# samuel-watson/glmmrMCML

Hardware: AMD Instinct MI355X
Metric: MCML iters/sec x m chains (simlik evals/sec) (higher is better)
Workload: dtype f64

## Files before the change

glmmrmcml_amd/csrc/debug_hooks.hip:

```cpp
#include "dgemm_mfma.h"
#include "dgemm_dl.h"
#include "dgemm_band.h"

using namespace mcml;

extern "C" int glmmr_mcml_dbg_dgemm(int M, int N, int K, const double* A, int lda,
                                    const double* B, int ldb, int b_nmajor,
                                    double alpha, double beta, double* C, int ldc,
                                    int lower_only, int force_tile)
{
    int ndev = 0;
    if (hipGetDeviceCount(&ndev) != hipSuccess || ndev == 0) {
        set_error("no HIP device: libglmmr_mcml_hip has no CPU fallback");
        return MCML_ENODEVICE;
    }
    hipStream_t s = nullptr;
    DevMat dA, dB, dC;
    if (force_tile == 40) {
        MCML_REQUIRE(!b_nmajor && !lower_only, "dbg_dgemm: the direct-to-LDS kernel takes a K-major B and all tiles");
        const int kpad = round_up(K, 32);
        MCML_TRY(dA.alloc(M, K, 32));
        MCML_HIP(hipMemset(dA.d(), 0, sizeof(double) * (size_t)dA.ld * dA.cols_alloc));
        MCML_HIP(hipMemcpy2D(dA.d(), sizeof(double) * dA.ld, A, sizeof(double) * lda, sizeof(double) * M, K, hipMemcpyHostToDevice));
        MCML_TRY(dB.alloc(kpad, N));
        MCML_HIP(hipMemset(dB.d(), 0, sizeof(double) * (size_t)dB.ld * N));
        MCML_HIP(hipMemcpy2D(dB.d(), sizeof(double) * dB.ld, B, sizeof(double) * ldb, sizeof(double) * K, N, hipMemcpyHostToDevice));
        MCML_TRY(upload_matrix(dC, C, M, N, ldc, s));
        MCML_REQUIRE(dlds_applicable(M, N, K, dA.d(), dA.ld, dA.cols_alloc, dB.d(), dB.ld), "dbg_dgemm: operands do not meet the direct-to-LDS contract");
        EpiAxpby epi2{dC.d(), dC.ld, alpha, beta};
        MCML_TRY(launch_gemm_dlds(s, M, N, K, dA.d(), dA.ld, dB.d(), dB.ld, epi2));
        MCML_TRY(download_matrix(C, ldc, dC.d(), dC.ld, M, N, s));
        return MCML_OK;
    }
    MCML_TRY(upload_matrix(dA, A, M, K, lda, s));
    if (b_nmajor) MCML_TRY(upload_matrix(dB, B, N, K, ldb, s));
    else MCML_TRY(upload_matrix(dB, B, K, N, ldb, s));
    MCML_TRY(upload_matrix(dC, C, M, N, ldc, s));
    EpiAxpby epi{dC.d(), dC.ld, alpha, beta};
    int rc;
    if (force_tile >= 20)
        rc = b_nmajor ? launch_gemm_dl<true>(s, M, N, K, dA.d(), dA.ld, dB.d(), dB.ld, epi, lower_only != 0, force_tile - 19)
                      : launch_gemm_dl<false>(s, M, N, K, dA.d(), dA.ld, dB.d(), dB.ld, epi, lower_only != 0, force_tile - 19);
    else
        rc = b_nmajor ? launch_gemm<true>(s, M, N, K, dA.d(), dA.ld, dB.d(), dB.ld, epi, lower_only != 0, force_tile)
                      : launch_gemm<false>(s, M, N, K, dA.d(), dA.ld, dB.d(), dB.ld, epi, lower_only != 0, force_tile);
    MCML_TRY(rc);
    MCML_TRY(download_matrix(C, ldc, dC.d(), dC.ld, M, N, s));
    return MCML_OK;
}

extern "C" int glmmr_mcml_dbg_dgemm_bench2(int M, int N, int K, int b_nmajor, int iters, int force_tile,
                                           int lower_only, double beta, double* ms_per_launch);
extern "C" int glmmr_mcml_dbg_dgemm_bench(int M, int N, int K, int b_nmajor, int iters,
                                          int force_tile, double* ms_per_launch)
{
    return glmmr_mcml_dbg_dgemm_bench2(M, N, K, b_nmajor, iters, force_tile, 0, 0.0, ms_per_launch);
}

extern "C" int glmmr_mcml_dbg_dgemm_bench2(int M, int N, int K, int b_nmajor, int iters, int force_tile,
                                           int lower_only, double beta, double* ms_per_launch)
{
    int ndev = 0;
    if (hipGetDeviceCount(&ndev) != hipSuccess || ndev == 0) {
        set_error("no HIP device: libglmmr_mcml_hip has no CPU fallback");
        return MCML_ENODEVICE;
    }
    hipStream_t s = nullptr;
    std::vector<double> hA((size_t)M * K), hB((size_t)K * N), hC((size_t)M * N, 0.0);
    uint64_t x = 88172645463325252ULL;
    auto rnd = [&]() { x ^= x << 13; x ^= x >> 7; x ^= x << 17; return (double)(x >> 11) / 9007199254740992.0 * 2 - 1; };
    for (auto& v : hA) v = rnd();
    for (auto& v : hB) v = rnd();
    DevMat dA, dB, dC;
    MCML_TRY(upload_matrix(dA, hA.data(), M, K, M, s));
    if (b_nmajor) MCML_TRY(upload_matrix(dB, hB.data(), N, K, N, s));
    else MCML_TRY(upload_matrix(dB, hB.data(), K, N, K, s));
    MCML_TRY(upload_matrix(dC, hC.data(), M, N, M, s));
    EpiAxpby epi{dC.d(), dC.ld, beta != 0.0 ? 1e-3 : 1.0, beta};
    const bool lo = lower_only != 0;
    auto go = [&]() {
        if (force_tile >= 20)
            return b_nmajor ? launch_gemm_dl<true>(s, M, N, K, dA.d(), dA.ld, dB.d(), dB.ld, epi, lo, force_tile - 19)
                            : launch_gemm_dl<false>(s, M, N, K, dA.d(), dA.ld, dB.d(), dB.ld, epi, lo, force_tile - 19);
        return b_nmajor ? launch_gemm<true>(s, M, N, K, dA.d(), dA.ld, dB.d(), dB.ld, epi, lo, force_tile)
                        : launch_gemm<false>(s, M, N, K, dA.d(), dA.ld, dB.d(), dB.ld, epi, lo, force_tile);
    };
    for (int i = 0; i < 3; i++) MCML_TRY(go());
    hipEvent_t e0, e1;
    MCML_HIP(hipEventCreate(&e0));
    MCML_HIP(hipEventCreate(&e1));
    MCML_HIP(hipEventRecord(e0, s));
    for (int i = 0; i < iters; i++) MCML_TRY(go());
    MCML_HIP(hipEventRecord(e1, s));
    MCML_HIP(hipEventSynchronize(e1));
    float ms = 0;
    MCML_HIP(hipEventElapsedTime(&ms, e0, e1));
    *ms_per_launch = ms / iters;
    (void)hipEventDestroy(e0);
    (void)hipEventDestroy(e1);
    return MCML_OK;
}

extern "C" int glmmr_mcml_dbg_dgemm_band(int M, int N, int K, const double* A, int lda, const double* B, int ldb,
                                         double* C, int ldc, int* tiles_executed)
{
    int ndev = 0;
    if (hipGetDeviceCount(&ndev) != hipSuccess || ndev == 0) {
        set_error("no HIP device: libglmmr_mcml_hip has no CPU fallback");
        return MCML_ENODEVICE;
    }
    MCML_REQUIRE(M > 0 && N > 0 && K > 0 && A && B && C, "dbg_dgemm_band: bad argument");
    hipStream_t s = nullptr;
    DevMat dA, dB, dC;
    MCML_TRY(dA.alloc(M, K, 32));
    MCML_HIP(hipMemset(dA.d(), 0, sizeof(double) * (size_t)dA.ld * dA.cols_alloc));
    MCML_HIP(hipMemcpy2D(dA.d(), sizeof(double) * dA.ld, A, sizeof(double) * lda, sizeof(double) * M, K, hipMemcpyHostToDevice));
    MCML_TRY(dB.alloc(round_up(K, 32), N));
    MCML_HIP(hipMemset(dB.d(), 0, sizeof(double) * (size_t)dB.ld * N));
    MCML_HIP(hipMemcpy2D(dB.d(), sizeof(double) * dB.ld, B, sizeof(double) * ldb, sizeof(double) * K, N, hipMemcpyHostToDevice));
    MCML_TRY(dC.alloc(M, N));
    MCML_HIP(hipMemset(dC.d(), 0, sizeof(double) * (size_t)dC.ld * N));
    MCML_REQUIRE(dlds_applicable(M, N, K, dA.d(), dA.ld, dA.cols_alloc, dB.d(), dB.ld), "dbg_dgemm_band: contract");
    const int nbands = (M + BD_BM - 1) / BD_BM;
    DevBuf kr;
    MCML_TRY(kr.ensure(sizeof(int) * 2 * nbands));
    hipLaunchKernelGGL(k_band_ranges, dim3(nbands), dim3(256), 0, s, dA.d(), dA.ld, M, K, kr.as<int>());
    MCML_HIP(hipGetLastError());
    std::vector<int> hk(2 * nbands);
    MCML_HIP(hipMemcpy(hk.data(), kr.p, sizeof(int) * 2 * nbands, hipMemcpyDeviceToHost));
    BandPlan plan;
    plan.reset(M, K, hk);
    if (tiles_executed) *tiles_executed = (int)plan.tiles;
    EpiAxpby epi{dC.d(), dC.ld, 1.0, 0.0};
    MCML_TRY(launch_gemm_band(s, plan, N, dA.d(), dA.ld, dB.d(), dB.ld, epi));
    MCML_TRY(download_matrix(C, ldc, dC.d(), dC.ld, M, N, s));
    return MCML_OK;
}

extern "C" int glmmr_mcml_dbg_band_clocks(int M, int N, int iters, int mode, double* out3)
{
    int ndev = 0;
    if (hipGetDeviceCount(&ndev) != hipSuccess || ndev == 0) {
        set_error("no HIP device: libglmmr_mcml_hip has no CPU fallback");
        return MCML_ENODEVICE;
    }
    hipStream_t s = nullptr;
    if (getenv("GLMMR_MCML_DBG_STREAM")) MCML_HIP(hipStreamCreateWithFlags(&s, hipStreamNonBlocking));
    std::vector<double> hA((size_t)M * M, 0.0), hB((size_t)M * N);
    uint64_t x = 88172645463325252ULL;
    auto rnd = [&]() { x ^= x << 13; x ^= x >> 7; x ^= x << 17; return (double)(x >> 11) / 9007199254740992.0 * 2 - 1; };
    const bool cst = getenv("GLMMR_MCML_DBG_DATA") && !strcmp(getenv("GLMMR_MCML_DBG_DATA"), "const");
    const bool dec = getenv("GLMMR_MCML_DBG_DATA") && !strcmp(getenv("GLMMR_MCML_DBG_DATA"), "decay");
    for (int j = 0; j < M; ++j) for (int i = j; i < M; ++i) hA[i + (size_t)j * M] = cst ? 1.0 : dec ? rnd() * std::exp(-(double)(i - j) / 40.0) : rnd();
    for (auto& v : hB) v = cst ? 1.0 : rnd();
    DevMat dA, dB, dC;
    MCML_TRY(dA.alloc(M, M, 32));
    MCML_HIP(hipMemset(dA.d(), 0, sizeof(double) * (size_t)dA.ld * dA.cols_alloc));
    MCML_HIP(hipMemcpy2D(dA.d(), sizeof(double) * dA.ld, hA.data(), sizeof(double) * M, sizeof(double) * M, M, hipMemcpyHostToDevice));
    MCML_TRY(dB.alloc(round_up(M, 32), N));
    MCML_HIP(hipMemset(dB.d(), 0, sizeof(double) * (size_t)dB.ld * N));
    MCML_HIP(hipMemcpy2D(dB.d(), sizeof(double) * dB.ld, hB.data(), sizeof(double) * M, sizeof(double) * M, N, hipMemcpyHostToDevice));
    MCML_TRY(dC.alloc(M, N));
    const int nbands = (M + BD_BM - 1) / BD_BM;
    DevBuf kr, clk;
    MCML_TRY(kr.ensure(sizeof(int) * 2 * nbands));
    MCML_TRY(clk.ensure(16));
    MCML_HIP(hipMemset(clk.p, 0, 16));
    hipLaunchKernelGGL(k_band_ranges, dim3(nbands), dim3(256), 0, s, dA.d(), dA.ld, M, M, kr.as<int>());
    std::vector<int> hk(2 * nbands);
    MCML_HIP(hipMemcpy(hk.data(), kr.p, sizeof(int) * 2 * nbands, hipMemcpyDeviceToHost));
    BandPlan plan;
    plan.reset(M, M, hk);
    const double tiles = (double)plan.tiles;
    EpiAxpby epi{dC.d(), dC.ld, 1.0, 0.0};
    if (mode < 0) {
        for (int i = 0; i < 3; i++)
            MCML_TRY((launch_gemm_band<EpiAxpby, false>(s, plan, N, dA.d(), dA.ld, dB.d(), dB.ld, epi)));
        hipEvent_t f0, f1;
        MCML_HIP(hipEventCreate(&f0));
        MCML_HIP(hipEventCreate(&f1));
        MCML_HIP(hipEventRecord(f0, s));
        for (int i = 0; i < iters; i++)
// ... 190 lines not shown
```

glmmrmcml_amd/csrc/dgemm_dl.h:

```cpp
#pragma once
#include "dgemm_dlds.h"

namespace mcml {

template <int WTM, int WTN, int WM, int WN, bool BNMAJOR, int STAGES>
struct DlgCfg {
    static constexpr int BK = 16;
    static constexpr int NW = WM * WN, THREADS = 64 * NW;
    static constexpr int BM = 16 * WTM * WM, BN = 16 * WTN * WN;
    static constexpr int A_BYTES = BK * BM * 8, B_BYTES = BK * BN * 8;
    static constexpr int A_CHUNKS = A_BYTES / 1024, B_CHUNKS = B_BYTES / 1024;
    static constexpr int CHUNKS = A_CHUNKS + B_CHUNKS;
    static constexpr int PER = (CHUNKS + NW - 1) / NW;
    static constexpr int STAGE_BYTES = A_BYTES + B_BYTES;
    static constexpr size_t LDS_BYTES = (size_t)STAGES * STAGE_BYTES;
    static constexpr bool SWZ_A = (BM % 32) == 0;
    static constexpr bool SWZ_B = BNMAJOR && (BN % 32) == 0;
    static_assert(BM % 8 == 0 && BN % 8 == 0, "tile sides are multiples of 8 doubles");
    static_assert(LDS_BYTES <= 160 * 1024, "LDS ring does not fit");
    static_assert(PER * (STAGES - 1) <= 24, "vmcnt immediates in dl_wait_vm");
};

template <int N>
__device__ __forceinline__ void dl_wait_vm()
{
#define MCML_VM(n) else if constexpr (N == n) asm volatile("s_waitcnt vmcnt(" #n ")" ::: "memory");
    if constexpr (N <= 0) asm volatile("s_waitcnt vmcnt(0)" ::: "memory");
    MCML_VM(1) MCML_VM(2) MCML_VM(3) MCML_VM(4) MCML_VM(5) MCML_VM(6) MCML_VM(7) MCML_VM(8)
    MCML_VM(9) MCML_VM(10) MCML_VM(11) MCML_VM(12) MCML_VM(13) MCML_VM(14) MCML_VM(15) MCML_VM(16)
    MCML_VM(17) MCML_VM(18) MCML_VM(19) MCML_VM(20) MCML_VM(21) MCML_VM(22) MCML_VM(23) MCML_VM(24)
    else asm volatile("s_waitcnt vmcnt(0)" ::: "memory");
#undef MCML_VM
}

template <int PER, int MAXT>
__device__ __forceinline__ void dl_wait_leave(int tiles)
{
    if constexpr (MAXT <= 0) dl_wait_vm<0>();
    else {
        if (tiles >= MAXT) dl_wait_vm<PER * MAXT>();
        else dl_wait_leave<PER, MAXT - 1>(tiles);
    }
}

template <int WTM, int WTN, int WM, int WN, bool BNMAJOR, int STAGES, class Epi>
__global__ __launch_bounds__(64 * WM * WN) void dgemm_dl_kernel(GemmP p, Epi epi)
{
    using Cfg = DlgCfg<WTM, WTN, WM, WN, BNMAJOR, STAGES>;
    constexpr int BM = Cfg::BM, BN = Cfg::BN, BK = Cfg::BK, NW = Cfg::NW, PER = Cfg::PER;
    extern __shared__ __attribute__((aligned(16))) double smem[];
    char* lds = reinterpret_cast<char*>(smem);
    const int tid = threadIdx.x, lane = tid & 63, wave = __builtin_amdgcn_readfirstlane(tid >> 6);
    const int wr = wave / WN, wc = wave - wr * WN;

    const int nblk = gridDim.x;
    const int bid = blockIdx.x;
    const int q8 = nblk >> 3, r8 = nblk & 7, xcd = bid & 7;
    const int nid = (xcd < r8 ? xcd * (q8 + 1) : r8 * (q8 + 1) + (xcd - r8) * q8) + (bid >> 3);
    int bi, bj;
    if (p.lower_only) {
        int rem = nid;
        for (bi = 0; bi < p.gm; ++bi) {
            int nc = (bi * BM + BM - 1 + p.diag_shift) / BN + 1;
            if (nc > p.gn) nc = p.gn;
            if (rem < nc) break;
            rem -= nc;
        }
        bj = rem;
    } else {
        bi = nid / p.gn; bj = nid - bi * p.gn;
    }
    const int m0 = bi * BM, n0 = bj * BN;

    unsigned voff[PER]; int loff[PER]; bool isA[PER];
#pragma unroll
    for (int s = 0; s < PER; ++s) {
        int c = wave + NW * s;
        if (c >= Cfg::CHUNKS) c = wave;
        isA[s] = c < Cfg::A_CHUNKS;
        if (c < Cfg::A_CHUNKS) {
            const int o = c * 1024 + lane * 16;
            const int k = o / (BM * 8), pos = (o - k * BM * 8) >> 3;
            const int m = Cfg::SWZ_A ? ((((pos >> 4) ^ (k & 1)) << 4) | (pos & 15)) : pos;
            int gm = m0 + m;
            if (gm >= p.M) gm = 0;
            voff[s] = (unsigned)((gm + (size_t)k * p.lda) * 8);
            loff[s] = c * 1024;
        } else {
            const int cb = c - Cfg::A_CHUNKS;
            const int o = cb * 1024 + lane * 16;
            if (BNMAJOR) {
                const int k = o / (BN * 8), pos = (o - k * BN * 8) >> 3;
                const int n = Cfg::SWZ_B ? ((((pos >> 4) ^ (k & 1)) << 4) | (pos & 15)) : pos;
                int gn = n0 + n;
                if (gn >= p.N) gn = 0;
                voff[s] = (unsigned)((gn + (size_t)k * p.ldb) * 8);
            } else {
                const int q = o >> 4;
                const int kp = q / BN, n = q - kp * BN;
                int gn = n0 + n;
                if (gn >= p.N) gn = 0;
                voff[s] = (unsigned)((2 * kp + (size_t)gn * p.ldb) * 8);
            }
            loff[s] = Cfg::A_BYTES + cb * 1024;
        }
    }
    const size_t stepA = (size_t)BK * p.lda * 8, stepB = BNMAJOR ? (size_t)BK * p.ldb * 8 : (size_t)BK * 8;
    const int by = blockIdx.y;
    const char* sA = reinterpret_cast<const char*>(p.A + (size_t)by * p.bsA);
    const char* sB = reinterpret_cast<const char*>(p.B + (size_t)by * p.bsB);

    auto issue = [&](int stage) {
        const unsigned lbase = (unsigned)(size_t)(lds_ptr_t)lds + stage * Cfg::STAGE_BYTES;
#pragma unroll
        for (int s = 0; s < PER; ++s) lds_dma16(lbase + loff[s], voff[s], isA[s] ? sA : sB);
        sA += stepA;
        sB += stepB;
    };

    d4 acc[WTM][WTN];
#pragma unroll
    for (int i = 0; i < WTM; ++i)
#pragma unroll
        for (int j = 0; j < WTN; ++j) acc[i][j] = d4{0.0, 0.0, 0.0, 0.0};

    const int l15 = lane & 15, lk = lane >> 4;
    auto compute = [&](int stage) {
        const double* as = reinterpret_cast<const double*>(lds + stage * Cfg::STAGE_BYTES);
        const double* bs = reinterpret_cast<const double*>(lds + stage * Cfg::STAGE_BYTES + Cfg::A_BYTES);
#pragma unroll
        for (int ks = 0; ks < BK / 4; ++ks) {
            const int kk = 4 * ks + lk;
            double a[WTM], b[WTN];
#pragma unroll
            for (int i = 0; i < WTM; ++i) {
                const int blk = wr * WTM + i;
                a[i] = as[kk * BM + ((Cfg::SWZ_A ? (blk ^ (kk & 1)) : blk) << 4) + l15];
            }
#pragma unroll
            for (int j = 0; j < WTN; ++j) {
                const int blk = wc * WTN + j;
                if (BNMAJOR) b[j] = bs[kk * BN + ((Cfg::SWZ_B ? (blk ^ (kk & 1)) : blk) << 4) + l15];
                else b[j] = bs[((kk >> 1) * BN + (blk << 4) + l15) * 2 + (kk & 1)];
            }
#pragma unroll
            for (int i = 0; i < WTM; ++i)
#pragma unroll
                for (int j = 0; j < WTN; ++j)
                    acc[i][j] = __builtin_amdgcn_mfma_f64_16x16x4f64(b[j], a[i], acc[i][j], 0, 0, 0);
        }
    };

    const int nk = p.K / BK;
    int issued = 0;
    for (; issued < STAGES - 1 && issued < nk; ++issued) issue(issued);
    dl_wait_leave<PER, STAGES - 2>(issued - 1);
    __builtin_amdgcn_s_barrier();
    int st = 0;
    for (int kt = 0; kt < nk; ++kt) {
        if (issued < nk) {
            int sn = st + STAGES - 1; if (sn >= STAGES) sn -= STAGES;
            issue(sn);
            ++issued;
        }
        compute(st);
        dl_wait_leave<PER, STAGES - 2>(issued - kt - 2);
        __builtin_amdgcn_s_barrier();
        st = st + 1; if (st >= STAGES) st = 0;
    }

    Epi e = epi;
    e.shift(by);
    e(acc, m0 + wr * 16 * WTM, n0 + wc * 16 * WTN, lane, p.M, p.N, bi * WM + wr);
}

static inline bool dl_applicable(int M, int N, int K, const double* A, int lda, const double* B, int ldb,
                                 bool bnmajor)
{
    return M >= 1 && N >= 1 && K >= 16 && (K & 15) == 0 && ((uintptr_t)A & 15) == 0 && ((uintptr_t)B & 15) == 0 &&
           (lda & 1) == 0 && (ldb & 1) == 0 && lda >= M && (bnmajor ? ldb >= N : ldb >= K) &&
           dma_offsets_fit((size_t)lda * 16 + M, bnmajor ? (size_t)ldb * 16 + N : (size_t)ldb * N + 16);
}

template <int WTM, int WTN, int WM, int WN, bool BNMAJOR, int STAGES, class Epi>
static inline int launch_gemm_dl_cfg(hipStream_t s, GemmP p, const Epi& epi, int nbatch = 1)
{
    using Cfg = DlgCfg<WTM, WTN, WM, WN, BNMAJOR, STAGES>;
    p.gm = (p.M + Cfg::BM - 1) / Cfg::BM;
    p.gn = (p.N + Cfg::BN - 1) / Cfg::BN;
    long ntiles = (long)p.gm * p.gn;
    if (p.lower_only) {
        ntiles = 0;
        for (int bi = 0; bi < p.gm; ++bi) {
            int nc = (bi * Cfg::BM + Cfg::BM - 1 + p.diag_shift) / Cfg::BN + 1;
            ntiles += nc > p.gn ? p.gn : nc;
        }
    }
    MCML_TRY(ensure_dynamic_lds(reinterpret_cast<const void*>(&dgemm_dl_kernel<WTM, WTN, WM, WN, BNMAJOR, STAGES, Epi>), (int)Cfg::LDS_BYTES));
    hipLaunchKernelGGL((dgemm_dl_kernel<WTM, WTN, WM, WN, BNMAJOR, STAGES, Epi>), dim3((unsigned)ntiles, (unsigned)nbatch),
                       dim3(Cfg::THREADS), Cfg::LDS_BYTES, s, p, epi);
    MCML_HIP(hipGetLastError());
    return MCML_OK;
}

constexpr int DL_TILE_BIG = 4, DL_TILE_SMALL = 5, DL_THR = 768, DL_THR64 = 128;

template <bool BNMAJOR, class Epi>
static inline int launch_gemm_dl(hipStream_t s, int M, int N, int K, const double* A, int lda,
                                 const double* B, int ldb, const Epi& epi, bool lower_only = false, int tile = 0,
                                 int inplace = 0, int diag_shift = 0, int nbatch = 1, size_t bsA = 0, size_t bsB = 0)
{
    MCML_REQUIRE(dl_applicable(M, N, K, A, lda, B, ldb, BNMAJOR), "dgemm_dl: shape/alignment contract violated "
                 "(M %d N %d K %d lda %d ldb %d)", M, N, K, lda, ldb);
    GemmP p{M, N, K, A, lda, B, ldb, 0, 0, lower_only ? 1 : 0, diag_shift, bsA, bsB};
    if (tile == 0) {
        long t128 = (long)((M + 127) / 128) * ((N + 127) / 128);
        if (lower_only) t128 = t128 / 2 + (M + 127) / 128;
        tile = t128 >= DL_THR ? DL_TILE_BIG : DL_TILE_SMALL;
        if (inplace == 0 && t128 < DL_THR64) tile = 6;
        if (inplace == 2) tile = N >= 256 ? 3 : 1;
    }
    MCML_REQUIRE(!(inplace == 1 && (tile == 6 || tile == 8) && N > (tile == 6 ? 64 : 32)) &&
                 !(inplace == 2 && (tile == 2 || tile == 5 || tile == 6 || tile == 7 || tile == 8) && M > (tile == 7 ? 16 : tile == 8 ? 32 : 64)),
                 "dgemm_dl: tile %d cannot run this product in place", tile);
    if (tile == 1) return launch_gemm_dl_cfg<4, 2, 2, 4, BNMAJOR, 4, Epi>(s, p, epi, nbatch);
    if (tile == 3) return launch_gemm_dl_cfg<1, 2, 8, 1, BNMAJOR, 6, Epi>(s, p, epi, nbatch);
    if (tile == 4) return launch_gemm_dl_cfg<4, 2, 2, 4, BNMAJOR, 2, Epi>(s, p, epi, nbatch);
    if (tile == 5) return launch_gemm_dl_cfg<2, 2, 2, 4, BNMAJOR, 3, Epi>(s, p, epi, nbatch);
    if (tile == 6) return launch_gemm_dl_cfg<2, 2, 2, 2, BNMAJOR, 3, Epi>(s, p, epi, nbatch);
    if (tile == 7) return launch_gemm_dl_cfg<1, 2, 1, 4, BNMAJOR, 4, Epi>(s, p, epi, nbatch);
    if (tile == 8) return launch_gemm_dl_cfg<1, 1, 2, 2, BNMAJOR, 4, Epi>(s, p, epi, nbatch);
    return launch_gemm_dl_cfg<2, 2, 2, 4, BNMAJOR, 5, Epi>(s, p, epi, nbatch);
}

}
```

glmmrmcml_amd/csrc/mvn.hip:

```cpp
#include "ctx.h"
#include "dgemm_mfma.h"
#include "dgemm_dl.h"
#include "reduce.h"

namespace mcml {

#define LOG_2PI 1.8378770664093454835606594728112

__global__ __launch_bounds__(256) void k_sum_partials(const double* partials, int n, double* out, int accumulate)
{
    __shared__ double sh[4];
    double v = 0;
    for (int i = threadIdx.x; i < n; i += 256) v += partials[i];
    double r = block_sum(v, sh);
    if (threadIdx.x == 0) out[0] = (accumulate ? out[0] : 0.0) + r;
}

int device_sum(Ctx& c, const double* partials, int n, double* dev_out)
{
    hipLaunchKernelGGL(k_sum_partials, dim3(1), dim3(256), 0, c.stream, partials, n, dev_out, 0);
    MCML_HIP(hipGetLastError());
    return MCML_OK;
}

__device__ __forceinline__ double diag_variance(const CovBlock& blk, const int32_t* cov, int rows, const ThetaArg& th)
{
    double val = 1.0;
    for (int r = blk.r0; r < blk.r1; ++r) val = cov_term(1, 0.0, &th.v[cov[r + 4 * rows]], val);
    return val;
}

__global__ void k_diag_prep(int Q, const int* rowblock, const CovBlock* blocks, const int32_t* cov,
                            int rows, ThetaArg th, double* dd, double* dc)
{
    int k = blockIdx.x * blockDim.x + threadIdx.x;
    if (k >= Q) return;
    int b = rowblock[k];
    if (b < 0) { dd[k] = 1.0; dc[k] = 0.0; return; }
    double d = sqrt(diag_variance(blocks[b], cov, rows, th));
    dd[k] = d * d;
    dc[k] = -0.5 * log(d * d) - 0.5 * LOG_2PI;
}

__global__ __launch_bounds__(256) void k_diag_ll(const double* U, int ldu, int Q, int mcols,
                                                 const int* rowblock, const double* dd,
                                                 const double* dc, double* partials)
{
    __shared__ double sh[4];
    int k = blockIdx.x * 256 + threadIdx.x;
    double acc = 0;
    if (k < Q && rowblock[k] >= 0) {
        const double idd = dd[k], c0 = dc[k];
        for (int col = blockIdx.y; col < mcols; col += gridDim.y) {
            double u = U[k + (size_t)col * ldu];
            acc += c0 - 0.5 * u * u / idd;
        }
    }
    double r = block_sum(acc, sh);
    if (threadIdx.x == 0) partials[blockIdx.y * gridDim.x + blockIdx.x] = r;
}

__device__ __forceinline__ double cov_entry(const CovBlock& blk, const int32_t* cov, int rows,
                                            const double* bd, const ThetaArg& th, int i, int j)
{
    double val = 1.0;
    int coff = 0;
    for (int r = blk.r0; r < blk.r1; ++r) {
        const int fn = cov[r + 2 * rows], nv = cov[r + 3 * rows], pi = cov[r + 4 * rows];
        double d2 = 0.0;
        for (int p = 0; p < nv; ++p) {
            double df = bd[i + (size_t)(coff + p) * blk.dim] - bd[j + (size_t)(coff + p) * blk.dim];
            d2 += df * df;
        }
        val = cov_term(fn, sqrt(d2), &th.v[pi], val);
        coff += nv;
    }
    return val;
}

__global__ __launch_bounds__(64) void k_small_ll(const double* U, int ldu, int mcols,
                                                 const int* small_ids, const CovBlock* blocks,
                                                 const int32_t* cov, int rows, const double* data,
                                                 ThetaArg th, double* partials, int* errflag)
{
    __shared__ double S[SMALL_BLOCK * (SMALL_BLOCK + 1)];
// ... 359 lines not shown
}

__global__ void k_copy_block(double* dst, int ldd, const double* src, int lds, int rows, int cols)
{
    int i = blockIdx.x * blockDim.x + threadIdx.x;
    if (i >= rows) return;
    for (int j = blockIdx.y; j < cols; j += gridDim.y) dst[i + (size_t)j * ldd] = src[i + (size_t)j * lds];
}

__global__ __launch_bounds__(256) void k_sumsq(const double* U, int ldu, int rows, int cols, double* partials)
{
    __shared__ double sh[4];
    int i = blockIdx.x * 256 + threadIdx.x;
    double acc = 0;
    if (i < rows)
        for (int j = blockIdx.y; j < cols; j += gridDim.y) {
            double u = U[i + (size_t)j * ldu];
            acc += u * u;
        }
    double r = block_sum(acc, sh);
    if (threadIdx.x == 0) partials[blockIdx.y * gridDim.x + blockIdx.x] = r;
}

__global__ __launch_bounds__(256) void k_logdet(const double* A, int lda, int n, double* out)
{
    __shared__ double sh[4];
    double acc = 0;
    for (int i = threadIdx.x; i < n; i += 256) acc += 2 * log(A[i + (size_t)i * lda]);
    double r = block_sum(acc, sh);
    if (threadIdx.x == 0) out[0] = r;
}

__global__ void k_finish_large(double* scal, int dim, int mcols)
{
    scal[0] += (double)mcols * (-0.5 * dim * LOG_2PI - 0.5 * scal[1]) - 0.5 * scal[2];
}

__global__ void k_zero_upper(double* A, int lda, int n)
{
    int i = blockIdx.x * blockDim.x + threadIdx.x;
    int j = blockIdx.y;
    if (i < n && j < n && i < j) A[i + (size_t)j * lda] = 0.0;
}

struct Bat { int n = 1; size_t sA = 0, sL = 0; int* err = nullptr; };

template <bool BNMAJOR>
static int chol_gemm(hipStream_t s, int M, int N, int K, const double* A, int lda, const double* B, int ldb,
                     const EpiAxpby& epi, bool lower_only, int tile, int inplace, int shift = 0, int nbatch = 1,
                     size_t bsA = 0, size_t bsB = 0)
{
    if (dl_applicable(M, N, K, A, lda, B, ldb, BNMAJOR))
        return launch_gemm_dl<BNMAJOR>(s, M, N, K, A, lda, B, ldb, epi, lower_only, tile, inplace, shift, nbatch, bsA, bsB);
    MCML_REQUIRE(nbatch == 1, "potrf: a batch of factorisations needs the LDS-DMA kernel for every panel product");
    MCML_REQUIRE(shift == 0 || !lower_only, "potrf: shifted lower-only update needs the LDS-DMA kernel");
    return launch_gemm<BNMAJOR>(s, M, N, K, A, lda, B, ldb, epi, lower_only, inplace ? inplace : -1);
}

static size_t linv_size(int n) { return (size_t)(n / CHOL_NB + 1) * CHOL_NB * CHOL_NB; }

static int leaf_prepare(Ctx& c, int n, int nbatch)
{
    const size_t bytes = sizeof(double) * linv_size(n) * nbatch;
    MCML_TRY(c.linv.ensure(bytes));
    MCML_HIP(hipMemsetAsync(c.linv.p, 0, bytes, c.stream));
    return ensure_dynamic_lds(reinterpret_cast<const void*>(&k_potrf_leaf<false>), (int)POTRF_LDS);
}

struct PotrfLaunch {
    Ctx& c; double* A; int lda; Bat bt; int* errflag;
    PotrfLaunch(Ctx& c_, double* A_, int lda_, const Bat& b)
        : c(c_), A(A_), lda(lda_), bt(b), errflag(b.err ? b.err : c_.errflag()) {}
    double* linv(int k) const { return c.linv.d() + (size_t)(k / CHOL_NB) * CHOL_NB * CHOL_NB; }
    int leaf(hipStream_t s, int k, int nb) const {
        hipLaunchKernelGGL(k_potrf_leaf<false>, dim3(bt.n), dim3(LEAF_NT), POTRF_LDS, s, A + k + (size_t)k * lda, lda, nb,
                           linv(k), errflag, bt.sA, bt.sL, LeafProf<false>());
        MCML_HIP(hipGetLastError());
        return MCML_OK;
    }
    int gemm_nt(hipStream_t s, int M, int N, int K, const double* Ap, const double* Bp, int ldb, double* Cp,
                double alpha, double beta, bool lower, int tile, int inplace, int shift) const {
        EpiAxpby epi{Cp, lda, alpha, beta, bt.sA};
        const size_t sB = (ldb == CHOL_NB) ? bt.sL : bt.sA;
        return chol_gemm<true>(s, M, N, K, Ap, lda, Bp, ldb, epi, lower, tile, inplace, shift, bt.n, bt.sA, sB);
    }
    struct Step { int k, nb, rem, R, nb2; double *A11, *A21; const double* Linv; };
    Step step(int t, int n, int extra) const {
        const int k = t * CHOL_NB, nb = (n - k < CHOL_NB) ? n - k : CHOL_NB, rem = n - k - nb;
        double* A11 = A + k + (size_t)k * lda;
        return Step{k, nb, rem, rem + extra, rem < CHOL_NB ? rem : CHOL_NB, A11, A11 + nb, linv(k)};
    }
};

static int lookahead_setup(Ctx& c)
{
    if (c.aux) return MCML_OK;
    int lo = 0, hi = 0;
    MCML_HIP(hipDeviceGetStreamPriorityRange(&lo, &hi));
    MCML_HIP(hipStreamCreateWithPriority(&c.aux, hipStreamNonBlocking, hi));
    MCML_HIP(hipStreamCreateWithPriority(&c.aux_lo, hipStreamNonBlocking, lo));
    MCML_HIP(hipEventCreateWithFlags(&c.ev_col, hipEventDisableTiming));
    MCML_HIP(hipEventCreateWithFlags(&c.ev_leaf, hipEventDisableTiming));
    return MCML_OK;
}

static int potrf_blocked(Ctx& c, double* A, int lda, int n, int extra, Bat bt = Bat())
{
    const PotrfLaunch L(c, A, lda, bt);
    const bool two = n > 2 * CHOL_NB;
    hipStream_t sM = c.stream, sL = c.stream;
    if (two) { MCML_TRY(lookahead_setup(c)); sL = c.aux; }
    const int nsteps = (n + CHOL_NB - 1) / CHOL_NB;
    constexpr int SPW = CHOL_NB * 8;
    const bool twolevel = bt.n > 1 && n > SPW + CHOL_NB;
    MCML_TRY(L.leaf(sM, 0, n < CHOL_NB ? n : CHOL_NB));
    bool forked = false;
    for (int t = 0; t < nsteps; ++t) {
        const PotrfLaunch::Step s = L.step(t, n, extra);
        const int k = s.k, nb = s.nb, rem = s.rem, R = s.R, nb2 = s.nb2;
        if (R <= 0) break;
        if (forked) { MCML_HIP(hipStreamWaitEvent(sM, c.ev_leaf, 0)); forked = false; }
        const int sp0 = twolevel ? (k / SPW) * SPW : 0, sp1 = twolevel ? (sp0 + SPW < n ? sp0 + SPW : n) : n;
        const int inner = sp1 - (k + nb);
        if (twolevel && inner == 0 && rem > 0) {
            MCML_TRY(L.gemm_nt(sM, R, nb, nb, s.A21, s.Linv, CHOL_NB, s.A21, 1.0, 0.0, false, 0, 1, 0));
            const double* Asp = A + sp1 + (size_t)sp0 * lda;
            double* Csp = A + sp1 + (size_t)sp1 * lda;
            MCML_TRY(L.gemm_nt(sM, R, rem, sp1 - sp0, Asp, Asp, lda, Csp, -1.0, 1.0, true, 0, 0, 0));
            MCML_TRY(L.leaf(sM, k + nb, nb2));
            continue;
        }
        if (nb2 > 0) {
            MCML_TRY(L.gemm_nt(sM, nb2, nb, nb, s.A21, s.Linv, CHOL_NB, s.A21, 1.0, 0.0, false, 7, 1, 0));
            double* T = s.A11 + nb + (size_t)nb * lda;
            MCML_TRY(L.gemm_nt(sM, nb2, nb2, nb, s.A21, s.A21, lda, T, -1.0, 1.0, false, 8, 0, 0));
            if (two) {
                MCML_HIP(hipEventRecord(c.ev_col, sM));
                MCML_HIP(hipStreamWaitEvent(sL, c.ev_col, 0));
            }
            MCML_TRY(L.leaf(sL, k + nb, nb2));
            if (two) { MCML_HIP(hipEventRecord(c.ev_leaf, sL)); forked = true; }
        }
        if (R - nb2 > 0)
            MCML_TRY(L.gemm_nt(sM, R - nb2, nb, nb, s.A21 + nb2, s.Linv, CHOL_NB, s.A21 + nb2, 1.0, 0.0, false, 0, 1, 0));
        if (rem > 0 && R - nb2 > 0) {
            double* C2 = s.A11 + nb + nb2 + (size_t)nb * lda;
            MCML_TRY(L.gemm_nt(sM, R - nb2, twolevel ? inner : rem, nb, s.A21 + nb2, s.A21, lda, C2, -1.0, 1.0, true, 0, 0, nb2));
        }
    }
    if (forked) MCML_HIP(hipStreamWaitEvent(sM, c.ev_leaf, 0));
    return MCML_OK;
}

static hipEvent_t ring_event(Ctx& c, size_t idx)
{
    while (c.ev_ring.size() <= idx) {
        hipEvent_t e = nullptr;
        if (hipEventCreateWithFlags(&e, hipEventDisableTiming) != hipSuccess) return nullptr;
        c.ev_ring.push_back(e);
    }
    return c.ev_ring[idx];
}
static int potrf_la2_capture(Ctx& c, double* A, int lda, int n, int extra, Bat bt = Bat())
{
    const PotrfLaunch L(c, A, lda, bt);
    hipStream_t sC = c.stream, sB = c.aux_lo;
// ... 448 lines not shown
```

include/glmmr_mcml_c.h:

```cpp
#ifndef GLMMR_MCML_C_H
#define GLMMR_MCML_C_H
#include <stdint.h>

#ifdef __cplusplus
extern "C" {
#endif

#define GLMMR_MCML_OK            0
#define GLMMR_MCML_EINVAL       -1
#define GLMMR_MCML_EUNSUPPORTED -2
#define GLMMR_MCML_ENOTPD       -3
#define GLMMR_MCML_ESINGULAR    -4
#define GLMMR_MCML_EHIP         -5
#define GLMMR_MCML_ENODEVICE    -6
#define GLMMR_MCML_ENOMEM       -7

const char* glmmr_mcml_last_error(void);


typedef struct glmmr_mcml_problem {
    const int32_t* cov;
    int            cov_rows;
    const double*  data;
    int            data_len;
// ... 134 lines not shown
                        double* theta, double* sigma, int* converged, int* iters,
                        glmmr_mcml_hmc_diag* last_diag);

int glmmr_mcml_full(const glmmr_mcml_problem* prob, const double* start, int nstart, int mcnr, int m,
                    int maxiter, int warmup, double tol, int verbose, double lambda, int trace,
                    int refresh, int maxsteps, double target_accept, const glmmr_mcml_ext* ext,
                    double* beta, double* theta, double* sigma, int* converged, double* u, int ldu,
                    int* ucols);

int glmmr_mcml_mcmc_sample(const double* Z, const double* L, const double* X, const double* y, int n,
                           int Q, int P, const double* beta, const char* family, const char* link,
                           int warmup, int nsamp, double lambda, double var_par, int trace, int refresh,
                           int maxsteps, double target_accept, const glmmr_mcml_ext* ext,
                           double* samples, int lds, int* ncols);

int glmmr_mcml_optim(const glmmr_mcml_problem* prob, const double* u, int ucols, const double* start,
                     int nstart, int trace, int mcnr, const glmmr_mcml_ext* ext, double* beta,
                     double* theta, double* sigma);
int glmmr_mcml_simlik(const glmmr_mcml_problem* prob, const double* u, int ucols, const double* start,
                      int nstart, int trace, const glmmr_mcml_ext* ext, double* beta, double* theta,
                      double* sigma);
int glmmr_mcml_optim_sparse(const glmmr_mcml_problem* prob, const int32_t* Ap, const int32_t* Ai, int nnz,
                            const double* u, int ucols, const double* start, int nstart, int trace,
                            int mcnr, const glmmr_mcml_ext* ext, double* beta, double* theta,
                            double* sigma,
                            int32_t* Lp, int32_t* Li, double* Lx, double* D, int lcap);
int glmmr_mcml_sparse_factor_nnz(const int32_t* cov, int cov_rows, const double* data, int data_len);
int glmmr_mcml_simlik_sparse(const glmmr_mcml_problem* prob, const int32_t* Ap, const int32_t* Ai, int nnz,
                             const double* u, int ucols, const double* start, int nstart, int trace,
                             const glmmr_mcml_ext* ext, double* beta, double* theta, double* sigma);
int glmmr_mcml_hess(const glmmr_mcml_problem* prob, const double* u, int ucols, const double* start,
                    int nstart, double tol, int trace, const glmmr_mcml_ext* ext, double* H);
int glmmr_mcml_hess_sparse(const glmmr_mcml_problem* prob, const int32_t* Ap, const int32_t* Ai, int nnz,
                           const double* u, int ucols, const double* start, int nstart, double tol,
                           int trace, const glmmr_mcml_ext* ext, double* H);
int glmmr_mcml_aic(const glmmr_mcml_problem* prob, const double* u, int ucols, const double* beta_par,
                   int nbeta, const double* cov_par, int ncov, const glmmr_mcml_ext* ext, double* out);

int glmmr_mcml_la(const glmmr_mcml_problem* prob, const double* start, int nstart, int usehess, double tol,
                  int verbose, int trace, int maxiter, const glmmr_mcml_ext* ext, double* beta, double* theta,
                  double* sigma, double* se, double* u);
int glmmr_mcml_la_nr(const glmmr_mcml_problem* prob, const double* start, int nstart, int usehess, double tol,
                     int verbose, int trace, int maxiter, const glmmr_mcml_ext* ext, double* beta, double* theta,
                     double* sigma, double* se, double* u);
int glmmr_mcml_ctx_la(glmmr_mcml_ctx* ctx, const double* start, int nstart, int nr, int usehess, double tol,
                      int verbose, int trace, int maxiter, const glmmr_mcml_ext* ext, double* beta, double* theta,
                      double* sigma, double* se, double* u, int* converged, int* iters);

int glmmr_mcml_mvn_ll(const int32_t* cov, int cov_rows, const double* data, int data_len,
                      const double* eff_range, int eff_len, const double* gamma, int ngamma,
                      const double* u, int Q, int m, double* out);

int glmmr_mcml_dbg_theta_log(glmmr_mcml_ctx* ctx, int enable, double* out, int cap_rows, int* nrows);
int glmmr_mcml_dbg_emulate_world(glmmr_mcml_ctx* ctx, int world, int mode);
int glmmr_mcml_dbg_leaf_profile(glmmr_mcml_ctx* ctx, unsigned long long* out10);
int glmmr_mcml_dbg_la_probe(glmmr_mcml_ctx* ctx, const double* start, int nstart, int kind, const double* v,
                            double var_par, const double* par, int npar, double* out, double* v_out,
                            double* beta_out, double* sigma_out);
int glmmr_mcml_dbg_dgemm(int M, int N, int K, const double* A, int lda, const double* B, int ldb,
                         int b_nmajor, double alpha, double beta, double* C, int ldc,
                         int lower_only, int force_tile );
int glmmr_mcml_dbg_log_prob_grad(glmmr_mcml_ctx* ctx, const double* beta, double var_par, const double* V,
                                 int ncols, double* lp, double* G);
int glmmr_mcml_dbg_normals(uint64_t seed, uint32_t chain, uint32_t prop, uint32_t tag, int n, double* out);
int glmmr_mcml_dbg_minstd(uint32_t seed, int n, double* out);
typedef double (*glmmr_mcml_objective)(const double* x, int n, void* user);
int glmmr_mcml_dbg_bobyqa(glmmr_mcml_objective f, void* user, int n, const double* x0, const double* lower,
                          const double* upper, double rhobeg, double rhoend, int maxfun, double* x_out,
                          double* f_out, int* nfev_out);
int glmmr_mcml_dbg_bobyqa_batch(glmmr_mcml_objective f, void* user, int n, const double* x0, const double* lower,
                                const double* upper, double rhobeg, double rhoend, int maxfun, int width,
                                double* x_out, double* f_out, int* nfev_out, int* rounds_out);
typedef int (*glmmr_mcml_batch_objective)(const double* X, int n, int k, double* F, void* user);
int glmmr_mcml_dbg_bobyqa_rounds(glmmr_mcml_batch_objective fb, void* user, int n, const double* x0, const double* lower,
                                 const double* upper, double rhobeg, double rhoend, int maxfun, int width,
                                 double* x_out, double* f_out, int* nfev_out, int* rounds_out);
int glmmr_mcml_dbg_copy_roundtrip(const double* in, long long ld_in, double* out, long long ld_out, long long rows, long long cols);
int glmmr_mcml_dbg_fd_hessian(glmmr_mcml_objective f, void* user, int n, const double* x, double ndeps,
                              int usebounds, const double* lower, const double* upper, double* H);
int glmmr_mcml_dbg_dgemm_bench(int M, int N, int K, int b_nmajor, int iters, int force_tile,
                               double* ms_per_launch);
int glmmr_mcml_dbg_dgemm_bench2(int M, int N, int K, int b_nmajor, int iters, int force_tile, int lower_only,
                                double beta, double* ms_per_launch);
int glmmr_mcml_dbg_dgemm_band(int M, int N, int K, const double* A, int lda, const double* B, int ldb, double* C,
                              int ldc, int* tiles_executed);
int glmmr_mcml_dbg_band_clocks(int M, int N, int iters, int mode, double* out3);

#ifdef __cplusplus
}
#endif
#endif
```

Baseline: 1123.

## Add dedicated long-K direct-to-LDS DGEMM kernel for Cholesky trailing updates

Adds a specialized 128x128 tile, 8-wave, 3-stage direct-to-LDS MFMA f64 GEMM kernel with double-buffered register reads of LDS fragments. The Cholesky batched GEMM path uses it when K exceeds the Cholesky block size and the update is not in-place, in place of the generic tile-selected kernel. The aim is better reuse and deeper pipelining of the long-K trailing updates. In exchange it adds fixed tile sizes that may underfill the GPU for small matrices. Tile mapping and tile counting are factored into shared helpers, and debug hooks are added.

```diff
diff --git a/glmmrmcml_amd/csrc/debug_hooks.hip b/glmmrmcml_amd/csrc/debug_hooks.hip
--- a/glmmrmcml_amd/csrc/debug_hooks.hip
+++ b/glmmrmcml_amd/csrc/debug_hooks.hip
@@ -1,5 +1,6 @@
 #include "dgemm_mfma.h"
 #include "dgemm_dl.h"
+#include "dgemm_bigk.h"
 #include "dgemm_band.h"
 
 using namespace mcml;
@@ -78,7 +79,13 @@
     MCML_TRY(upload_matrix(dC, hC.data(), M, N, M, s));
     EpiAxpby epi{dC.d(), dC.ld, beta != 0.0 ? 1e-3 : 1.0, beta};
     const bool lo = lower_only != 0;
-    auto go = [&]() {
+    MCML_REQUIRE(force_tile != 30 || b_nmajor, "dbg_dgemm_bench: the long-K kernel takes an N-major B");
+    MCML_REQUIRE(force_tile != 40 || (!b_nmajor && !lo && dlds_applicable(M, N, K, dA.d(), dA.ld, dA.cols_alloc, dB.d(), dB.ld)),
+                 "dbg_dgemm_bench: the direct-to-LDS kernel takes a K-major B, all tiles and K a multiple of 32");
+    auto go = [&]() -> int {
+        if (force_tile == 40) return launch_gemm_dlds(s, M, N, K, dA.d(), dA.ld, dB.d(), dB.ld, epi);
+        if (force_tile == 30)
+            return launch_gemm_bigk(s, M, N, K, dA.d(), dA.ld, dB.d(), dB.ld, epi, lo);
         if (force_tile >= 20)
             return b_nmajor ? launch_gemm_dl<true>(s, M, N, K, dA.d(), dA.ld, dB.d(), dB.ld, epi, lo, force_tile - 19)
                             : launch_gemm_dl<false>(s, M, N, K, dA.d(), dA.ld, dB.d(), dB.ld, epi, lo, force_tile - 19);
@@ -98,6 +105,33 @@
     *ms_per_launch = ms / iters;
     (void)hipEventDestroy(e0);
     (void)hipEventDestroy(e1);
+    return MCML_OK;
+}
+
+extern "C" int glmmr_mcml_dbg_dgemm_bigk(double* W, int ld, int ncols, int nbatch, int M, int N, int K, int a_row,
+                                         int b_row, int k_col, int c_row, int c_col, double alpha, double beta,
+                                         int lower_only, int diag_shift, int kernel)
+{
+    int ndev = 0;
+    if (hipGetDeviceCount(&ndev) != hipSuccess || ndev == 0) {
+        set_error("no HIP device: libglmmr_mcml_hip has no CPU fallback");
+        return MCML_ENODEVICE;
+    }
+    MCML_REQUIRE(W && ld > 0 && ncols > 0 && nbatch >= 1 && M > 0 && N > 0 && K > 0 && a_row >= 0 && b_row >= 0 &&
+                 k_col >= 0 && c_row >= 0 && c_col >= 0 && a_row + M <= ld && b_row + N <= ld && c_row + M <= ld &&
+                 k_col + K <= ncols && c_col + N <= ncols, "dbg_dgemm_bigk: operands outside the workspace");
+    hipStream_t s = nullptr;
+    const size_t per = (size_t)ld * ncols;
+    DevBuf buf;
+    MCML_TRY(buf.ensure(sizeof(double) * per * nbatch));
+    MCML_TRY(copy_h2d(buf.p, W, sizeof(double) * per * nbatch, s));
+    const double* A = buf.d() + a_row + (size_t)k_col * ld;
+    const double* B = buf.d() + b_row + (size_t)k_col * ld;
+    EpiAxpby epi{buf.d() + c_row + (size_t)c_col * ld, ld, alpha, beta, per};
+    if (kernel < 0) MCML_TRY(launch_gemm_bigk(s, M, N, K, A, ld, B, ld, epi, lower_only != 0, diag_shift, nbatch, per, per));
+    else MCML_TRY(launch_gemm_dl<true>(s, M, N, K, A, ld, B, ld, epi, lower_only != 0, kernel, 0, diag_shift, nbatch, per, per));
+    MCML_TRY(copy_d2h(W, buf.p, sizeof(double) * per * nbatch, s));
+    MCML_HIP(hipStreamSynchronize(s));
     return MCML_OK;
 }
 
diff --git a/glmmrmcml_amd/csrc/dgemm_bigk.h b/glmmrmcml_amd/csrc/dgemm_bigk.h
--- /dev/null
+++ b/glmmrmcml_amd/csrc/dgemm_bigk.h
@@ -0,0 +1,150 @@
+#pragma once
+#include "dgemm_dl.h"
+
+namespace mcml {
+
+struct BkCfg {
+    static constexpr int BM = 128, BN = 128, BK = 16, STAGES = 3;
+    static constexpr int A_BYTES = BK * BM * 8, STAGE_BYTES = A_BYTES + BK * BN * 8;
+    static constexpr size_t LDS_BYTES = (size_t)STAGES * STAGE_BYTES;
+    static constexpr int PER = 4;
+};
+
+template <int KS>
+__device__ __forceinline__ void bk_read(double (&a)[4], double (&b)[2], unsigned ae, unsigned ao, unsigned be, unsigned bo)
+{
+    DL_RD(a[0], ae, KS * 4 * BkCfg::BM * 8);
+    DL_RD(a[1], ao, KS * 4 * BkCfg::BM * 8 + 128);
+    DL_RD(a[2], ae, KS * 4 * BkCfg::BM * 8 + 256);
+    DL_RD(a[3], ao, KS * 4 * BkCfg::BM * 8 + 384);
+    DL_RD(b[0], be, KS * 4 * BkCfg::BN * 8);
+    DL_RD(b[1], bo, KS * 4 * BkCfg::BN * 8 + 128);
+}
+template <int LEAVE>
+__device__ __forceinline__ void bk_wait(double (&a)[4], double (&b)[2])
+{
+#if defined(__HIP_DEVICE_COMPILE__)
+    if constexpr (LEAVE == 6)
+        asm volatile("s_waitcnt lgkmcnt(6)" : "+v"(a[0]), "+v"(a[1]), "+v"(a[2]), "+v"(a[3]), "+v"(b[0]), "+v"(b[1]));
+    else
+        asm volatile("s_waitcnt lgkmcnt(0)" : "+v"(a[0]), "+v"(a[1]), "+v"(a[2]), "+v"(a[3]), "+v"(b[0]), "+v"(b[1]));
+#endif
+}
+__device__ __forceinline__ void bk_mfma(d4 (&acc)[4][2], const double (&a)[4], const double (&b)[2])
+{
+#pragma unroll
+    for (int i = 0; i < 4; ++i)
+#pragma unroll
+        for (int j = 0; j < 2; ++j) acc[i][j] = __builtin_amdgcn_mfma_f64_16x16x4f64(b[j], a[i], acc[i][j], 0, 0, 0);
+}
+
+template <class Epi>
+__global__ __launch_bounds__(512) void dgemm_bigk_kernel(GemmP p, Epi epi)
+{
+    using Cfg = BkCfg;
+    constexpr int BM = Cfg::BM, BN = Cfg::BN, BK = Cfg::BK, STAGES = Cfg::STAGES, PER = Cfg::PER;
+    extern __shared__ __attribute__((aligned(16))) double smem[];
+    char* lds = reinterpret_cast<char*>(smem);
+    const int tid = threadIdx.x, lane = tid & 63, wave = __builtin_amdgcn_readfirstlane(tid >> 6);
+    const int wr = wave >> 2, wc = wave & 3;
+
+    int bi, bj;
+    dl_tile_of<BM, BN>(p, bi, bj);
+    const int m0 = bi * BM, n0 = bj * BN;
+
+    unsigned voff[PER];
+    {
+        const int pos = 2 * lane, m = ((((pos >> 4) ^ (wave & 1)) << 4) | (pos & 15));
+        int gm = m0 + m, gn = n0 + m;
+        if (gm >= p.M) gm = 0;
+        if (gn >= p.N) gn = 0;
+#pragma unroll
+        for (int s = 0; s < 2; ++s) {
+            const int k = wave + 8 * s;
+            voff[s] = (unsigned)((gm + (size_t)k * p.lda) * 8);
+            voff[2 + s] = (unsigned)((gn + (size_t)k * p.ldb) * 8);
+        }
+    }
+    const size_t stepA = (size_t)BK * p.lda * 8, stepB = (size_t)BK * p.ldb * 8;
+    const int by = blockIdx.y;
+    const char* sA = reinterpret_cast<const char*>(p.A + (size_t)by * p.bsA);
+    const char* sB = reinterpret_cast<const char*>(p.B + (size_t)by * p.bsB);
+    const unsigned lds0 = (unsigned)(size_t)(lds_ptr_t)lds;
+    auto issue = [&](int stage) {
+        const unsigned lbase = lds0 + stage * Cfg::STAGE_BYTES + wave * 1024;
+        lds_dma16(lbase, voff[0], sA);
+        lds_dma16(lbase + 8 * 1024, voff[1], sA);
+        lds_dma16(lbase + Cfg::A_BYTES, voff[2], sB);
+        lds_dma16(lbase + Cfg::A_BYTES + 8 * 1024, voff[3], sB);
+        sA += stepA;
+        sB += stepB;
+    };
+
+    d4 acc[4][2];
+#pragma unroll
+    for (int i = 0; i < 4; ++i)
+#pragma unroll
+        for (int j = 0; j < 2; ++j) acc[i][j] = d4{0.0, 0.0, 0.0, 0.0};
+
+    const int l15 = lane & 15, lk = lane >> 4, par = lk & 1;
+    const unsigned abase = lds0 + lk * (BM * 8) + l15 * 8 + wr * 4 * 128;
+    const unsigned bbase = lds0 + Cfg::A_BYTES + lk * (BN * 8) + l15 * 8 + wc * 2 * 128;
+    const unsigned a_even = abase + par * 128, a_odd = abase - par * 128;
+    const unsigned b_even = bbase + par * 128, b_odd = bbase - par * 128;
+
+    const int nk = p.K / BK;
+    int issued = 0;
+    for (; issued < STAGES - 1 && issued < nk; ++issued) issue(issued);
+    dl_wait_leave<PER, STAGES - 2>(issued - 1);
+    __builtin_amdgcn_s_barrier();
+    int st = 0;
+    double ra[2][4], rb[2][2];
+    bk_read<0>(ra[0], rb[0], a_even, a_odd, b_even, b_odd);
+    for (int kt = 0; kt < nk; ++kt) {
+        if (issued < nk) {
+            int sn = st + STAGES - 1; if (sn >= STAGES) sn -= STAGES;
+            issue(sn);
+            ++issued;
+        }
+        const unsigned so = st * Cfg::STAGE_BYTES;
+        int stn = st + 1; if (stn >= STAGES) stn = 0;
+#define BK_STEP(KS, CUR, NXT)                                                                    \
+        bk_read<KS + 1>(ra[NXT], rb[NXT], a_even + so, a_odd + so, b_even + so, b_odd + so);      \
+        bk_wait<6>(ra[CUR], rb[CUR]);                                                             \
+        bk_mfma(acc, ra[CUR], rb[CUR]);                                                           \
+        __builtin_amdgcn_sched_barrier(0);
+        BK_STEP(0, 0, 1) BK_STEP(1, 1, 0) BK_STEP(2, 0, 1)
+#undef BK_STEP
+        dl_wait_leave<PER, STAGES - 2>(issued - kt - 2);
+        bk_wait<0>(ra[1], rb[1]);
+        __builtin_amdgcn_s_barrier();
+        if (kt + 1 < nk) {
+            const unsigned sn2 = stn * Cfg::STAGE_BYTES;
+            bk_read<0>(ra[0], rb[0], a_even + sn2, a_odd + sn2, b_even + sn2, b_odd + sn2);
+        }
+        bk_mfma(acc, ra[1], rb[1]);
+        __builtin_amdgcn_sched_barrier(0);
+        st = stn;
+    }
+
+    Epi e = epi;
+    e.shift(by);
+    e(acc, m0 + wr * 64, n0 + wc * 32, lane, p.M, p.N, bi * 2 + wr);
+}
+
+template <class Epi>
+static inline int launch_gemm_bigk(hipStream_t s, int M, int N, int K, const double* A, int lda, const double* B,
+                                   int ldb, const Epi& epi, bool lower_only, int diag_shift = 0, int nbatch = 1,
+                                   size_t bsA = 0, size_t bsB = 0)
+{
+    MCML_REQUIRE(dl_applicable(M, N, K, A, lda, B, ldb, true), "dgemm_bigk: shape/alignment contract violated "
+                 "(M %d N %d K %d lda %d ldb %d)", M, N, K, lda, ldb);
+    GemmP p{M, N, K, A, lda, B, ldb, 0, 0, lower_only ? 1 : 0, diag_shift, bsA, bsB};
+    const long ntiles = dl_count_tiles<BkCfg::BM, BkCfg::BN>(p);
+    MCML_TRY(ensure_dynamic_lds(reinterpret_cast<const void*>(&dgemm_bigk_kernel<Epi>), (int)BkCfg::LDS_BYTES));
+    hipLaunchKernelGGL((dgemm_bigk_kernel<Epi>), dim3((unsigned)ntiles, (unsigned)nbatch), dim3(512), BkCfg::LDS_BYTES, s, p, epi);
+    MCML_HIP(hipGetLastError());
+    return MCML_OK;
+}
+
+}
diff --git a/glmmrmcml_amd/csrc/dgemm_dl.h b/glmmrmcml_amd/csrc/dgemm_dl.h
--- a/glmmrmcml_amd/csrc/dgemm_dl.h
+++ b/glmmrmcml_amd/csrc/dgemm_dl.h
@@ -43,21 +43,13 @@
     }
 }
 
-template <int WTM, int WTN, int WM, int WN, bool BNMAJOR, int STAGES, class Epi>
-__global__ __launch_bounds__(64 * WM * WN) void dgemm_dl_kernel(GemmP p, Epi epi)
-{
-    using Cfg = DlgCfg<WTM, WTN, WM, WN, BNMAJOR, STAGES>;
-    constexpr int BM = Cfg::BM, BN = Cfg::BN, BK = Cfg::BK, NW = Cfg::NW, PER = Cfg::PER;
-    extern __shared__ __attribute__((aligned(16))) double smem[];
-    char* lds = reinterpret_cast<char*>(smem);
-    const int tid = threadIdx.x, lane = tid & 63, wave = __builtin_amdgcn_readfirstlane(tid >> 6);
-    const int wr = wave / WN, wc = wave - wr * WN;
-
+template <int BM, int BN>
+__device__ __forceinline__ void dl_tile_of(const GemmP& p, int& bi, int& bj)
+{
     const int nblk = gridDim.x;
     const int bid = blockIdx.x;
     const int q8 = nblk >> 3, r8 = nblk & 7, xcd = bid & 7;
     const int nid = (xcd < r8 ? xcd * (q8 + 1) : r8 * (q8 + 1) + (xcd - r8) * q8) + (bid >> 3);
-    int bi, bj;
     if (p.lower_only) {
         int rem = nid;
         for (bi = 0; bi < p.gm; ++bi) {
@@ -70,6 +62,33 @@
     } else {
         bi = nid / p.gn; bj = nid - bi * p.gn;
     }
+}
+template <int BM, int BN>
+static inline long dl_count_tiles(GemmP& p)
+{
+    p.gm = (p.M + BM - 1) / BM;
+    p.gn = (p.N + BN - 1) / BN;
+    if (!p.lower_only) return (long)p.gm * p.gn;
+    long ntiles = 0;
+    for (int bi = 0; bi < p.gm; ++bi) {
+        int nc = (bi * BM + BM - 1 + p.diag_shift) / BN + 1;
+        ntiles += nc > p.gn ? p.gn : nc;
+    }
+    return ntiles;
+}
+
+template <int WTM, int WTN, int WM, int WN, bool BNMAJOR, int STAGES, class Epi>
+__global__ __launch_bounds__(64 * WM * WN) void dgemm_dl_kernel(GemmP p, Epi epi)
+{
+    using Cfg = DlgCfg<WTM, WTN, WM, WN, BNMAJOR, STAGES>;
+    constexpr int BM = Cfg::BM, BN = Cfg::BN, BK = Cfg::BK, NW = Cfg::NW, PER = Cfg::PER;
+    extern __shared__ __attribute__((aligned(16))) double smem[];
+    char* lds = reinterpret_cast<char*>(smem);
+    const int tid = threadIdx.x, lane = tid & 63, wave = __builtin_amdgcn_readfirstlane(tid >> 6);
+    const int wr = wave / WN, wc = wave - wr * WN;
+
+    int bi, bj;
+    dl_tile_of<BM, BN>(p, bi, bj);
     const int m0 = bi * BM, n0 = bj * BN;
 
     unsigned voff[PER]; int loff[PER]; bool isA[PER];
@@ -186,16 +205,7 @@
 static inline int launch_gemm_dl_cfg(hipStream_t s, GemmP p, const Epi& epi, int nbatch = 1)
 {
     using Cfg = DlgCfg<WTM, WTN, WM, WN, BNMAJOR, STAGES>;
-    p.gm = (p.M + Cfg::BM - 1) / Cfg::BM;
-    p.gn = (p.N + Cfg::BN - 1) / Cfg::BN;
-    long ntiles = (long)p.gm * p.gn;
-    if (p.lower_only) {
-        ntiles = 0;
-        for (int bi = 0; bi < p.gm; ++bi) {
-            int nc = (bi * Cfg::BM + Cfg::BM - 1 + p.diag_shift) / Cfg::BN + 1;
-            ntiles += nc > p.gn ? p.gn : nc;
-        }
-    }
+    const long ntiles = dl_count_tiles<Cfg::BM, Cfg::BN>(p);
     MCML_TRY(ensure_dynamic_lds(reinterpret_cast<const void*>(&dgemm_dl_kernel<WTM, WTN, WM, WN, BNMAJOR, STAGES, Epi>), (int)Cfg::LDS_BYTES));
     hipLaunchKernelGGL((dgemm_dl_kernel<WTM, WTN, WM, WN, BNMAJOR, STAGES, Epi>), dim3((unsigned)ntiles, (unsigned)nbatch),
                        dim3(Cfg::THREADS), Cfg::LDS_BYTES, s, p, epi);
diff --git a/glmmrmcml_amd/csrc/mvn.hip b/glmmrmcml_amd/csrc/mvn.hip
--- a/glmmrmcml_amd/csrc/mvn.hip
+++ b/glmmrmcml_amd/csrc/mvn.hip
@@ -1,6 +1,7 @@
 #include "ctx.h"
 #include "dgemm_mfma.h"
 #include "dgemm_dl.h"
+#include "dgemm_bigk.h"
 #include "reduce.h"
 
 namespace mcml {
@@ -526,6 +527,8 @@
                 double alpha, double beta, bool lower, int tile, int inplace, int shift) const {
         EpiAxpby epi{Cp, lda, alpha, beta, bt.sA};
         const size_t sB = (ldb == CHOL_NB) ? bt.sL : bt.sA;
+        if (K > CHOL_NB && inplace == 0 && dl_applicable(M, N, K, Ap, lda, Bp, ldb, true))
+            return launch_gemm_bigk(s, M, N, K, Ap, lda, Bp, ldb, epi, lower, shift, bt.n, bt.sA, sB);
         return chol_gemm<true>(s, M, N, K, Ap, lda, Bp, ldb, epi, lower, tile, inplace, shift, bt.n, bt.sA, sB);
     }
     struct Step { int k, nb, rem, R, nb2; double *A11, *A21; const double* Linv; };
diff --git a/include/glmmr_mcml_c.h b/include/glmmr_mcml_c.h
--- a/include/glmmr_mcml_c.h
+++ b/include/glmmr_mcml_c.h
@@ -240,6 +240,9 @@
                                double* ms_per_launch);
 int glmmr_mcml_dbg_dgemm_bench2(int M, int N, int K, int b_nmajor, int iters, int force_tile, int lower_only,
                                 double beta, double* ms_per_launch);
+int glmmr_mcml_dbg_dgemm_bigk(double* W, int ld, int ncols, int nbatch, int M, int N, int K, int a_row, int b_row,
+                              int k_col, int c_row, int c_col, double alpha, double beta, int lower_only, int diag_shift,
+                              int kernel);
 int glmmr_mcml_dbg_dgemm_band(int M, int N, int K, const double* A, int lda, const double* B, int ldb, double* C,
                               int ldc, int* tiles_executed);
 int glmmr_mcml_dbg_band_clocks(int M, int N, int iters, int mode, double* out3);
```

New measurement: 1122. About the same (-0.1%).
